# tomershay100/mp3-steganography-lib

Measured on AMD Instinct MI355X. Metric: MP3 frames/sec (decode+re-encode) @44.1kHz stereo 128kbps, 1→8 GPU, higher is better.
Workload: dtype f64 (decode) / int32 (encode); 1 GPU; 10000-frame full decode->stego-embed->re-encode pipeline per MI355X (BASELINE configs[2]); MP3 main data + side info resident in HBM, MP3 frames out; the message cursor chain is decided and the serial chains of the rate loop are checked on the device inside every step; frames_per_gpu=10000, channels=2, message_bits=536, chain_verdict_units_to_redo=0, message_variant_entries=1874, parallelism=frames sharded over 1 GPU(s), no collective

## Files before the change

include/mp3s.h:

```cpp
#ifndef MP3S_H
#define MP3S_H
#include <stddef.h>
#include <stdint.h>

#ifdef __cplusplus
extern "C" {
#endif

#define MP3S_OK 0
#define MP3S_E_NO_DEVICE (-1)
#define MP3S_E_HIP (-2)
#define MP3S_E_ARG (-3)
#define MP3S_E_MALFORMED (-4)
#define MP3S_E_UNSUPPORTED (-5)
#define MP3S_E_STEP_RANGE (-6)
#define MP3S_E_NOMEM (-7)
#define MP3S_E_EXIT (-8)
#define MP3S_E_BUSY (-9)
#define MP3S_E_TABLES (-10)

#define MP3S_PCM_I16 0
#define MP3S_PCM_F32 1
#define MP3S_PCM_F64 2

// ... 95 lines not shown
int mp3s_debug_walk_rate(const uint8_t *file, size_t len, double seconds, double *frames_per_s, int64_t *frames_per_pass);

int mp3s_dev_alloc(mp3s_ctx *ctx, size_t bytes, void **dptr);
int mp3s_dev_free(mp3s_ctx *ctx, void *dptr);
int mp3s_dev_upload(mp3s_ctx *ctx, void *dptr, const void *host, size_t bytes);
int mp3s_dev_download(mp3s_ctx *ctx, void *host, const void *dptr, size_t bytes);
int mp3s_dev_memset(mp3s_ctx *ctx, void *dptr, int value, size_t bytes);
int mp3s_dev_copy(mp3s_ctx *ctx, void *d_dst, const void *d_src, size_t bytes);
int mp3s_timer_start(mp3s_ctx *ctx);
int mp3s_timer_stop(mp3s_ctx *ctx, float *ms);
int mp3s_synth_mode(mp3s_ctx *ctx, double eps_scale, int64_t *exact_samples);
int mp3s_bench_copy(mp3s_ctx *ctx, size_t bytes, int iters, double *gb_per_s);
#define MP3S_N_KERNELS 9
#define MP3S_N_KERNELS_MIN 8
int mp3s_profile_enable(mp3s_ctx *ctx, int on);
int mp3s_profile_select(mp3s_ctx *ctx, unsigned mask);
int mp3s_profile_collect(mp3s_ctx *ctx, double *total_ms, int64_t *launches, int n);

int mp3s_decode_transform_dev(mp3s_ctx *ctx, const int16_t *d_is, const mp3s_granule_si *d_si,
                              const mp3s_frame_hdr *d_hdr, int n_frames, int nch, int n_halo, int out_format,
                              void *d_pcm);
int mp3s_decode_transform(mp3s_ctx *ctx, const int16_t *is, const mp3s_granule_si *si, const mp3s_frame_hdr *hdr,
                          int n_frames, int nch, int n_halo, int out_format, void *pcm);

int mp3s_encode_transform_dev(mp3s_ctx *ctx, const int16_t *d_pcm, const mp3s_frame_hdr *d_hdr, int n_frames,
                              int32_t *d_mdct);
int mp3s_encode_transform(mp3s_ctx *ctx, const int16_t *pcm, const mp3s_frame_hdr *hdr, int n_frames,
                          int32_t *mdct);

int mp3s_rate_loop_dev(mp3s_ctx *ctx, const int32_t *d_mdct, const mp3s_rate_frame *d_frames, int n_frames,
                       const uint8_t *d_hide_bits, int n_hide, const int32_t *d_cursor_in, const int32_t *d_state_in,
                       const int32_t *d_unit_list, int n_list, int16_t *d_ix, mp3s_gr_out *d_out, int32_t *d_en);

typedef struct {
    int32_t first_frame, n_frames;
    int32_t hide_base;
    int32_t hide_begin;
    int32_t hide_end;
    int32_t reserved;
    int32_t chain_in[4][4];
} mp3s_chain_seg;
typedef struct {
    int64_t cursor;
    int32_t chain[4][4];
    int32_t carry_used;
    int32_t reserved;
} mp3s_chain_seg_out;
int mp3s_chain_resolve_dev(mp3s_ctx *ctx, mp3s_gr_out *d_gr, const mp3s_rate_frame *d_frames, int n_frames,
                           const mp3s_chain_seg *d_segs, int n_segs, const int32_t *d_cursor_in, const int32_t *d_state_in,
                           int32_t *d_verdict, mp3s_chain_seg_out *d_seg_out);

int mp3s_chain_redo_dev(mp3s_ctx *ctx, const int32_t *d_mdct, const mp3s_rate_frame *d_frames, int n_frames,
                        const uint8_t *d_hide_bits, int n_hide, int32_t *d_cursor, const mp3s_chain_seg *d_segs, int n_segs,
                        int16_t *d_ix, mp3s_gr_out *d_gr, int32_t *d_en, int32_t *d_verdict, mp3s_chain_seg_out *d_seg_out);

#define MP3S_SELECT_VARIANTS 10
#define MP3S_SELECT_TAIL_FIRST(bits_left, reach) ((bits_left) < 2 ? 0 : (((bits_left) - 2) / 3 < (reach) ? ((bits_left) - 2) / 3 : (reach)))
#define MP3S_SELECT_ENTRIES(bits_left, reach) (8 * (reach) + 2 * ((reach) - MP3S_SELECT_TAIL_FIRST(bits_left, reach)))
#define MP3S_SELECT_MAX_REACH (1 << 18)
#define MP3S_NO_CURSOR 0x3fffffff
typedef struct {
    int32_t first_entry;
    int32_t reach;
} mp3s_select_span;
void mp3s_select_patterns(uint8_t out[32]);
int mp3s_select_plan(const mp3s_chain_seg *segs, int n_segs, mp3s_select_span *spans, int32_t *ent_unit, int32_t *ent_cursor, int cap);
// ... 298 lines not shown
```

mp3-steganography-lib_amd/csrc/k_chain.hpp:

```cpp
#pragma once

namespace mp3s {

constexpr int CH_THREADS = 256;

struct ChainEl { int reset, tables, last[4]; };

__device__ __forceinline__ ChainEl chain_identity() { return ChainEl{0, 0, {-1, -1, -1, -1}}; }
__device__ __forceinline__ ChainEl chain_combine(const ChainEl &l, const ChainEl &r)
{
    if (r.reset) return r;
    ChainEl o;
    o.reset = l.reset;
    o.tables = l.tables + r.tables;
#pragma unroll
    for (int k = 0; k < 4; k++) o.last[k] = r.last[k] >= 0 ? r.last[k] : l.last[k];
    return o;
}
__device__ __forceinline__ ChainEl chain_shfl_up(const ChainEl &x, int d)
{
    ChainEl o;
    o.reset = __shfl_up(x.reset, d, 64);
    o.tables = __shfl_up(x.tables, d, 64);
#pragma unroll
    for (int k = 0; k < 4; k++) o.last[k] = __shfl_up(x.last[k], d, 64);
    return o;
}

__device__ __forceinline__ ChainEl chain_block_scan(ChainEl x, ChainEl (&wave_tot)[CH_THREADS / 64], ChainEl *total)
{
    const int lane = threadIdx.x & 63, wave = threadIdx.x >> 6;
#pragma unroll
    for (int d = 1; d < 64; d <<= 1) {
        const ChainEl o = chain_shfl_up(x, d);
        if (lane >= d) x = chain_combine(o, x);
    }
    __syncthreads();
    if (lane == 63) wave_tot[wave] = x;
    __syncthreads();
    ChainEl pre = chain_identity();
#pragma unroll
    for (int w = 0; w < CH_THREADS / 64; w++) {
        if (w < wave) pre = chain_combine(pre, wave_tot[w]);
    }
    x = chain_combine(pre, x);
    if (total) {
        ChainEl t = wave_tot[0];
#pragma unroll
        for (int w = 1; w < CH_THREADS / 64; w++) t = chain_combine(t, wave_tot[w]);
        *total = t;
    }
    return x;
}

__device__ __forceinline__ ChainEl chain_element(const mp3s_gr_out *__restrict__ gr, const mp3s_rate_frame *__restrict__ rf,
                                                 const mp3s_chain_seg *__restrict__ segs, int f, int n_frames)
{
    ChainEl e = chain_identity();
    if (f >= n_frames) return e;
    e.reset = segs[rf[f].stream].first_frame == f ? 1 : 0;
#pragma unroll
    for (int k = 0; k < 4; k++) {
        const mp3s_gr_out &g = gr[(long)f * 4 + k];
        if (g.flags & MP3S_RF_ACTIVE) { e.tables += g.n_tables; e.last[k] = f * 4 + k; }
    }
    return e;
}

__global__ __launch_bounds__(CH_THREADS) void k_chain_sum(const mp3s_gr_out *__restrict__ gr, const mp3s_rate_frame *__restrict__ rf,
                                                          const mp3s_chain_seg *__restrict__ segs, int n_frames,
                                                          ChainEl *__restrict__ agg, int32_t *__restrict__ verdict,
                                                          mp3s_chain_seg_out *__restrict__ seg_out, int32_t *__restrict__ redo,
                                                          const int32_t *__restrict__ only_after)
{
    __shared__ ChainEl wave_tot[CH_THREADS / 64];
    if (only_after && only_after[0] == 0) {
        if (redo && blockIdx.x == 0 && threadIdx.x == 0) redo[0] = 0;
        return;
    }
    const int f = blockIdx.x * CH_THREADS + threadIdx.x;
    if (f == 0) { verdict[0] = 0; verdict[1] = 0; }
    if (redo) {
        if (f == 0) redo[0] = 0;
        if (f == 0 && !only_after) redo[REDO_WORDS] = 0;
    }
    if (f < n_frames && segs[rf[f].stream].first_frame == f) seg_out[rf[f].stream].carry_used = 0;
    ChainEl total;
    chain_block_scan(chain_element(gr, rf, segs, f, n_frames), wave_tot, &total);
    if (threadIdx.x == 0) agg[blockIdx.x] = total;
}

__global__ __launch_bounds__(CH_THREADS) void k_chain_apply(mp3s_gr_out *__restrict__ gr, const mp3s_rate_frame *__restrict__ rf,
                                                            const mp3s_chain_seg *__restrict__ segs, int n_frames,
                                                            const ChainEl *__restrict__ agg, int32_t *__restrict__ cursor_in,
                                                            const int32_t *__restrict__ state_in, int32_t *__restrict__ verdict,
                                                            mp3s_chain_seg_out *__restrict__ seg_out, int32_t *__restrict__ redo_list,
                                                            const int32_t *__restrict__ only_after)
{
    if (only_after && only_after[0] == 0) return;
    __shared__ ChainEl wave_tot[CH_THREADS / 64];
    const int f = blockIdx.x * CH_THREADS + threadIdx.x;
    ChainEl before = chain_identity();
    for (int c0 = 0; c0 < (int)blockIdx.x; c0 += CH_THREADS) {
        const int j = c0 + (int)threadIdx.x;
        ChainEl total;
        chain_block_scan(j < (int)blockIdx.x ? agg[j] : chain_identity(), wave_tot, &total);
        before = chain_combine(before, total);
    }
    const ChainEl own_el = chain_element(gr, rf, segs, f, n_frames);
    const ChainEl incl = chain_block_scan(own_el, wave_tot, nullptr);
    ChainEl excl = chain_shfl_up(incl, 1);
    if ((threadIdx.x & 63) == 0) {
        excl = chain_identity();
        for (int w = 0; w < (int)(threadIdx.x >> 6); w++) excl = chain_combine(excl, wave_tot[w]);
    }
    excl = chain_combine(before, excl);
    int redo_here = 0, err_here = 0;
    if (f < n_frames) {
        const int s = rf[f].stream;
        const mp3s_chain_seg sg = segs[s];
        const bool first = sg.first_frame == f;
        if (first) excl = chain_identity();
        long cur = (long)sg.hide_begin + excl.tables;
        const long end = sg.hide_end;
        const bool hiding = sg.hide_end > sg.hide_base;
        int carry_used = first && cur < end ? 1 : 0;
#pragma unroll
        for (int k = 0; k < 4; k++) {
            const long u = (long)f * 4 + k;
            mp3s_gr_out &g = gr[u];
            int32_t ch[4];
            const bool own = excl.last[k] >= 0;
            if (own) {
                const mp3s_gr_out &p = gr[excl.last[k]];
                ch[0] = p.address[0]; ch[1] = p.address[1]; ch[2] = p.address[2]; ch[3] = p.quantizer_step;
            } else {
#pragma unroll
                for (int j = 0; j < 4; j++) ch[j] = sg.chain_in[k][j];
            }
            const int flags = g.flags;
            const bool active = flags & MP3S_RF_ACTIVE;
            if (!own && (!active || (flags & MP3S_RF_USED_ADDR_IN))) carry_used = 1;
            bool redo = false;
            if (hiding && active) {
                const long used = cursor_in[u];
                if (used != cur && (used < cur ? used : cur) < end) redo = true;
            }
            if (flags & MP3S_RF_USED_ADDR_IN) {
                const int32_t given = state_in ? state_in[u * 4] | (state_in[u * 4 + 1] << 10) | (state_in[u * 4 + 2] << 20) : g.reserved0;
                if (given != (ch[0] | (ch[1] << 10) | (ch[2] << 20))) redo = true;
            }
            redo_here += redo ? 1 : 0;
            if (redo && redo_list) {
                const int at = atomicAdd(&redo_list[0], 1);
                if (at < REDO_CAP) {
                    const int32_t c = (int32_t)(cur < (long)MP3S_NO_CURSOR ? cur : (long)MP3S_NO_CURSOR);
                    redo_list[REDO_HEAD + at] = (int32_t)u;
                    g.flags = flags | MP3S_RF_LISTED;
                    redo_list[REDO_HEAD + REDO_CAP + at] = hiding ? c : (cursor_in ? cursor_in[u] : 0);
                    if (hiding) cursor_in[u] = c;
#pragma unroll
                    for (int j = 0; j < 4; j++) redo_list[REDO_HEAD + 2 * REDO_CAP + 4 * at + j] = ch[j];
                }
            } else if (flags & MP3S_RF_LISTED) {
                g.flags = flags & ~MP3S_RF_LISTED;
            }
            if (flags & MP3S_RF_STEP_RANGE) err_here = 1;
            if (active) cur += g.n_tables;
            else {
                g.address[0] = ch[0]; g.address[1] = ch[1]; g.address[2] = ch[2];
                g.quantizer_step = ch[3];
            }
        }
        if (carry_used) atomicOr(&seg_out[s].carry_used, 1);
        if (f == sg.first_frame + sg.n_frames - 1) {
            seg_out[s].cursor = cur;
#pragma unroll
            for (int k = 0; k < 4; k++) {
                const mp3s_gr_out &g = gr[(long)f * 4 + k];
                seg_out[s].chain[k][0] = g.address[0]; seg_out[s].chain[k][1] = g.address[1];
                seg_out[s].chain[k][2] = g.address[2]; seg_out[s].chain[k][3] = g.quantizer_step;
            }
        }
    }
    const int n_redo = (int)wave_add_u32((uint32_t)redo_here);
    const bool any_err = __ballot(err_here != 0) != 0;
    if ((threadIdx.x & 63) == 0) {
        if (n_redo) atomicAdd(&verdict[0], n_redo);
        if (any_err) atomicOr(&verdict[1], 1);
    }
}

constexpr int SEL_THREADS = 1024, SEL_WAVES = SEL_THREADS / 64, SEL_D = 128;
constexpr int SEL_ROUND = SEL_THREADS;
constexpr int SEL_SAFE = 32;
constexpr int SEL_NONE = MP3S_SELECT_VARIANTS;

__host__ __device__ inline size_t select_lds_bytes(int reach)
{
    const int rs = reach < SEL_ROUND ? reach : SEL_ROUND;
    return (size_t)rs * (SEL_NONE + 1) + (size_t)(3 * rs + SEL_D + 8) + (size_t)rs + SEL_WAVES * SEL_D + 64;
}

__global__ __launch_bounds__(SEL_THREADS) void k_chain_select(const mp3s_chain_seg *__restrict__ segs, const mp3s_select_span *__restrict__ spans,
                                                              int max_reach, const uint8_t *__restrict__ hide,
                                                              const uint8_t *__restrict__ tabv, const mp3s_gr_out *__restrict__ out,
                                                              int32_t *__restrict__ cursor, int2 *__restrict__ pairs)
{
    extern __shared__ uint8_t sel_lds[];
    __shared__ int overflow, d_next, d_try, sat_round;
    const int s = blockIdx.x;
    const mp3s_select_span sp = spans[s];
    const int R = sp.reach;
    const int tid = threadIdx.x, lane = tid & 63, wave = __builtin_amdgcn_readfirstlane(tid >> 6);
    int2 *my_pairs = pairs + (long)s * max_reach;
    if (R <= 0) {
        for (int j = tid; j < max_reach; j += SEL_THREADS) my_pairs[j] = make_int2(-1, 0);
        return;
    }
    const mp3s_chain_seg sg = segs[s];
    const long c0 = sg.hide_begin, end = sg.hide_end;
    const long u0 = (long)sg.first_frame * 4;
    const int RS = min(R, SEL_ROUND);
    const long left = end - c0;
    const int tail = (int)MP3S_SELECT_TAIL_FIRST(left, (long)R), R2 = R - tail;
    const long row8 = (long)sp.first_entry + 8L * R - tail;
    uint8_t *tabs = sel_lds;
    uint8_t *code = tabs + (size_t)RS * (SEL_NONE + 1);
    uint8_t *delta = code + 3 * RS + SEL_D + 8;
    uint8_t *tot = delta + RS;
    if (tid == 0) { overflow = 0; d_next = 0; }
    int size = SEL_ROUND;
    for (int J = 0; J < R;) {
        __syncthreads();
        if (tid == 0) sat_round = 0;
        const int Rs = min(size, R - J);
        const int d0 = d_next;
        const long rel0 = 3L * J - d0 - (SEL_D - 1);
        if (c0 + rel0 >= end) {
            for (int jj = tid; jj < Rs; jj += SEL_THREADS) my_pairs[J + jj] = make_int2(-1, 0);
// ... 38 lines not shown
                d = step(jj, d);
            }
            if (sat && lane == 0) sat_round = 1;
            if (wave == SEL_WAVES - 1 && lane == 0) d_try = d0 + d;
        }
        __syncthreads();
        if (sat_round) {
            if (size > SEL_SAFE) { size = SEL_SAFE; continue; }
            if (tid == 0) overflow = 1;
        }
        for (int jj = tid; jj < Rs; jj += SEL_THREADS) {
            const int p = 3 * jj + (SEL_D - 1) - (int)delta[jj];
            const int v = code[p];
            const int j = J + jj;
            if (v >= 8 && v != SEL_NONE && j < tail) overflow = 1;
            my_pairs[j] = v == SEL_NONE ? make_int2(-1, 0)
                                        : make_int2(v < 8 ? sp.first_entry + v * R + j : (int)(row8 + (long)(v - 8) * R2 + j), (int)(rel0 + p));
        }
        if (tid == 0) d_next = d_try;
        J += Rs;
        if (size == SEL_SAFE && J % SEL_ROUND == 0) size = SEL_ROUND;
    }
    __syncthreads();
    const bool bad = overflow != 0;
    for (int j = tid; j < max_reach; j += SEL_THREADS) {
        int src = -1;
        if (j < R && !bad) {
            const int2 pr = my_pairs[j];
            src = pr.x;
            if (src >= 0) cursor[u0 + j] = (int32_t)(c0 + pr.y);
        }
        my_pairs[j] = make_int2(src, (int)(u0 + j));
    }
}

}
```

mp3-steganography-lib_amd/csrc/k_rate.hpp:

```cpp
#pragma once
#ifndef MP3S_RL_STATS
#define MP3S_RL_STATS 0
#endif
#ifndef MP3S_RL_OCC
#define MP3S_RL_OCC 6
#endif
#if MP3S_RL_STATS
__device__ unsigned long long g_rl_stats[128];
extern "C" __attribute__((visibility("default"))) int mp3s_debug_rl_stats(unsigned long long *out, int clear)
{
    (void)hipDeviceSynchronize();
    int rc = (int)hipMemcpyFromSymbol(out, HIP_SYMBOL(g_rl_stats), sizeof(unsigned long long) * 128);
    if (clear) { unsigned long long z[128] = {}; rc |= (int)hipMemcpyToSymbol(HIP_SYMBOL(g_rl_stats), z, sizeof z); }
    return rc;
}
#define RL_STAT(i, v) do { if ((threadIdx.x & 63) == 0) atomicAdd(&g_rl_stats[(i)], (unsigned long long)(v)); } while (0)
#define RL_CLK() __builtin_readcyclecounter()
#else
#define RL_STAT(i, v) do { } while (0)
#endif

namespace mp3s {

#define RL_DPP(v, ctrl, rm) ((uint32_t)__builtin_amdgcn_update_dpp(0, (int)(v), ctrl, rm, 0xf, false))
// ... 610 lines not shown
        if (!CHAIN) break;
        ch_state[0] = __builtin_amdgcn_readfirstlane(st.a1); ch_state[1] = __builtin_amdgcn_readfirstlane(st.a2);
        ch_state[2] = __builtin_amdgcn_readfirstlane(st.a3); ch_state[3] = __builtin_amdgcn_readfirstlane(qstep);
        bool go = false;
        int un = u;
        for (;;) {
            un += 4;
            if (++steps >= REDO_CHAIN_MAX || un >= n_units || frames[un >> 2].stream != fr.stream) break;
            const int f2 = __builtin_amdgcn_readfirstlane(__hip_atomic_load(&out[un - out_base].flags, __ATOMIC_RELAXED, __HIP_MEMORY_SCOPE_AGENT));
            if (f2 & MP3S_RF_LISTED) break;
            if (!(f2 & MP3S_RF_ACTIVE)) continue;
            const int given = __builtin_amdgcn_readfirstlane(__hip_atomic_load(&out[un - out_base].reserved0, __ATOMIC_RELAXED, __HIP_MEMORY_SCOPE_AGENT));
            go = (f2 & MP3S_RF_USED_ADDR_IN) && given != (ch_state[0] | (ch_state[1] << 10) | (ch_state[2] << 20));
            break;
        }
        if (!go) break;
        u = un; chained = true;
        ch_cursor = (n_hide_all > 0 && cursor_all) ? cursor_all[u] : 0;
    }
    }
    } while (CHAIN && (li0 += (int)gridDim.x * RL_WAVES) < n_total);
}

__global__ __launch_bounds__(RL_WAVES * 64, MP3S_RL_OCC) void k_rate_loop(
    const int32_t *__restrict__ mdct, const mp3s_rate_frame *__restrict__ frames, int n_units,
    const uint8_t *__restrict__ hide, int n_hide, const int32_t *__restrict__ cursor_in,
    const int32_t *__restrict__ state_in, const int32_t *__restrict__ unit_list, int n_list,
    int16_t *__restrict__ ix_out, mp3s_gr_out *__restrict__ out, int32_t *__restrict__ en_out, int out_base, int compact,
    RateVariants var)
{
    rate_units(mdct, frames, n_units, hide, n_hide, cursor_in, state_in, unit_list, n_list, ix_out, out, en_out, out_base, compact, var);
}

__global__ __launch_bounds__(RL_WAVES * 64, 4) void k_rate_redo(
    const int32_t *__restrict__ mdct, const mp3s_rate_frame *__restrict__ frames, int n_units,
    const uint8_t *__restrict__ hide, int n_hide, const int32_t *__restrict__ redo, int16_t *__restrict__ ix_out,
    mp3s_gr_out *__restrict__ out, int32_t *__restrict__ en_out, const int32_t *__restrict__ cursor_all)
{
    const int32_t *unit_list = redo + REDO_HEAD;
    const int n_list = min(__builtin_amdgcn_readfirstlane(__hip_atomic_load(&redo[0], __ATOMIC_RELAXED, __HIP_MEMORY_SCOPE_AGENT)), REDO_CAP);
    if ((int)blockIdx.x * RL_WAVES >= n_list) return;
    const RateVariants none = {nullptr, nullptr, 0, nullptr, nullptr, nullptr, nullptr};
    rate_units<true>(mdct, frames, n_units, hide, n_hide, unit_list + REDO_CAP, unit_list + 2 * REDO_CAP, unit_list, n_list, ix_out, out, en_out,
                  0, 3, none, cursor_all);
}

__global__ __launch_bounds__(256) void k_gather_tables(const mp3s_gr_out *__restrict__ outv, int n, uint8_t *__restrict__ tables)
{
    const int i = blockIdx.x * 256 + threadIdx.x;
    if (i < n) tables[i] = (uint8_t)outv[i].n_tables;
}

__global__ __launch_bounds__(256) void k_scatter_entries(const int2 *__restrict__ pairs, int n_pairs, const int16_t *__restrict__ ixv,
                                                         const int32_t *__restrict__ env, const mp3s_gr_out *__restrict__ outv,
                                                         int16_t *__restrict__ ix, int32_t *__restrict__ en, mp3s_gr_out *__restrict__ out)
{
    const int wave = __builtin_amdgcn_readfirstlane(threadIdx.x >> 6), lane = threadIdx.x & 63;
    const int j = blockIdx.x * 4 + wave;
    if (j >= n_pairs) return;
    const int2 pr = pairs[j];
    if (pr.x < 0) return;
    const long src = pr.x, dst = pr.y;
    const uint32_t *a = reinterpret_cast<const uint32_t *>(ixv + src * 576);
    uint32_t *b = reinterpret_cast<uint32_t *>(ix + dst * 576);
    for (int i = lane; i < 288; i += 64) b[i] = a[i];
    if (lane < 22) en[dst * 22 + lane] = env[src * 22 + lane];
    static_assert(sizeof(mp3s_gr_out) % 4 == 0, "GrInfo is copied by words");
    if (lane < (int)(sizeof(mp3s_gr_out) / 4))
        reinterpret_cast<uint32_t *>(out + dst)[lane] = reinterpret_cast<const uint32_t *>(outv + src)[lane];
}

}
```

mp3-steganography-lib_amd/csrc/mp3s_device.hip:

```cpp
#include <hip/hip_runtime.h>
#include <hip/hip_ext.h>
#include <atomic>
#include <stdint.h>
#include <stdlib.h>

#include "../../include/mp3s.h"
#include "mp3s_device.h"
#include "mp3s_host.h"
#include "mp3s_tables.h"

namespace mp3s {
__constant__ DevTables c_tab;
}

#include "k_sync.hpp"
#include "k_decode.hpp"
#include "k_decode_stream.hpp"
#include "k_encode.hpp"
#include "k_rate.hpp"
#include "k_huffman.hpp"
#include "k_parse.hpp"
#include "k_reveal.hpp"
#include "k_capacity.hpp"
#include "k_pack.hpp"
// ... 164 lines not shown
    hipLaunchKernelGGL(k_enc_analysis, dim3((unsigned)((waves + 3) / 4)), dim3(256), 0, stream, d_pcm, d_hdr, n_frames, SB,
                       Ts);
    if (prof) prof->end(stream, pp);
    pp = prof ? prof->begin(stream, K_ENC_MDCT) : -1;
    hipLaunchKernelGGL(k_enc_mdct, dim3((n_frames + 3) / 4), dim3(256), 0, stream, (const int32_t *)SB, Ts, d_hdr, n_frames,
                       d_mdct);
    if (prof) prof->end(stream, pp);
    return (int)hipGetLastError();
}

int launch_rate(hipStream_t stream, const int32_t *d_mdct, const mp3s_rate_frame *d_frames, int n_frames,
                const uint8_t *d_hide, int n_hide, const int32_t *d_cursor, const int32_t *d_state,
                const int32_t *d_list, int n_list, int16_t *d_ix, mp3s_gr_out *d_out, int32_t *d_en, Profiler *prof, int out_base, int compact,
                const RateVariantArgs *variants, hipEvent_t done)
{
    const int n_units = n_frames * 4;
    if (compact && !d_list) return (int)hipErrorInvalidValue;
    const int n = d_list ? n_list : n_units;
    RateVariants var = {nullptr, nullptr, 0, nullptr, nullptr, nullptr, nullptr};
    if (variants && variants->n > 0) var = RateVariants{variants->d_unit, variants->d_cursor, variants->n, variants->d_ix, variants->d_out, variants->d_en, variants->d_tables};
    if (n + var.n <= 0) return done ? (int)hipEventRecord(done, stream) : 0;
    hipEvent_t t_start = nullptr, t_stop = nullptr;
    const bool timed = prof && prof->attach(K_RATE_LOOP, &t_start, &t_stop);
    if (timed || done)
        hipExtLaunchKernelGGL(k_rate_loop, dim3((n + var.n + RL_WAVES - 1) / RL_WAVES), dim3(RL_WAVES * 64), 0, stream, timed ? t_start : nullptr, timed ? t_stop : done, 0,
                              d_mdct, d_frames, n_units, d_hide, n_hide, d_cursor, d_state, d_list, n, d_ix, d_out, d_en, out_base, compact, var);
    else
        hipLaunchKernelGGL(k_rate_loop, dim3((n + var.n + RL_WAVES - 1) / RL_WAVES), dim3(RL_WAVES * 64), 0, stream, d_mdct, d_frames,
                           n_units, d_hide, n_hide, d_cursor, d_state, d_list, n, d_ix, d_out, d_en, out_base, compact, var);
    if (timed && done && hipEventRecord(done, stream) != hipSuccess) return (int)hipErrorUnknown;
    return (int)hipGetLastError();
}

static size_t chain_scan_bytes(int n_frames) { return ((size_t)((n_frames + CH_THREADS - 1) / CH_THREADS) * sizeof(ChainEl) + 31) & ~(size_t)15; }
constexpr int kRedoRounds = 1;
size_t chain_agg_bytes(int n_frames) { return chain_scan_bytes(n_frames) + (size_t)2 * REDO_WORDS * 4; }

int launch_chain(hipStream_t stream, mp3s_gr_out *d_gr, const mp3s_rate_frame *d_frames, int n_frames, const mp3s_chain_seg *d_segs,
                 const int32_t *d_cursor, const int32_t *d_state, void *d_agg, int32_t *d_verdict, mp3s_chain_seg_out *d_seg_out,
                 Profiler *prof, const ChainRedoArgs *redo)
{
    if (n_frames <= 0) return 0;
    const int blocks = (n_frames + CH_THREADS - 1) / CH_THREADS;
    int32_t *d_redo = redo ? (int32_t *)((uint8_t *)d_agg + chain_scan_bytes(n_frames)) : nullptr;
    int32_t *cursor = const_cast<int32_t *>(d_cursor);
    const int pp = prof ? prof->begin(stream, K_CHAIN) : -1;
    hipLaunchKernelGGL(k_chain_sum, dim3(blocks), dim3(CH_THREADS), 0, stream, (const mp3s_gr_out *)d_gr, d_frames, d_segs, n_frames,
                       (ChainEl *)d_agg, d_verdict, d_seg_out, d_redo, (const int32_t *)nullptr);
    hipLaunchKernelGGL(k_chain_apply, dim3(blocks), dim3(CH_THREADS), 0, stream, d_gr, d_frames, d_segs, n_frames,
                       (const ChainEl *)d_agg, cursor, d_state, d_verdict, d_seg_out, d_redo, (const int32_t *)nullptr);
    if (redo) {
        int32_t *lists[2] = {d_redo, d_redo + REDO_WORDS};
        for (int round = 0; round < kRedoRounds; round++) {
            const int32_t *cur = lists[round & 1];
            int32_t *nxt = round + 1 < kRedoRounds ? lists[(round + 1) & 1] : nullptr;
            hipLaunchKernelGGL(k_rate_redo, dim3(REDO_GROUPS), dim3(RL_WAVES * 64), 0, stream, redo->d_mdct, d_frames, n_frames * 4,
                               redo->d_hide, redo->n_hide, cur, redo->d_ix, d_gr, redo->d_en, (const int32_t *)d_cursor);
            hipLaunchKernelGGL(k_chain_sum, dim3(blocks), dim3(CH_THREADS), 0, stream, (const mp3s_gr_out *)d_gr, d_frames, d_segs, n_frames,
                               (ChainEl *)d_agg, d_verdict, d_seg_out, nxt, cur);
            hipLaunchKernelGGL(k_chain_apply, dim3(blocks), dim3(CH_THREADS), 0, stream, d_gr, d_frames, d_segs, n_frames,
                               (const ChainEl *)d_agg, cursor, d_state, d_verdict, d_seg_out, nxt, cur);
        }
    }
    if (prof) prof->end(stream, pp);
    return (int)hipGetLastError();
}

int launch_select(hipStream_t stream, const mp3s_chain_seg *d_segs, const mp3s_select_span *d_spans, int n_segs, int max_reach,
                  const uint8_t *d_hide, const RateVariantArgs &v, int16_t *d_ix, int32_t *d_en, mp3s_gr_out *d_out, int32_t *d_cursor,
                  void *d_pairs, Profiler *prof)
{
    if (n_segs <= 0 || max_reach <= 0 || v.n <= 0) return 0;
    if (max_reach > MP3S_SELECT_MAX_REACH || (int64_t)n_segs * max_reach > 0x3fffffff) return (int)hipErrorInvalidValue;
    const int pp = prof ? prof->begin(stream, K_CHAIN) : -1;
    hipLaunchKernelGGL(k_chain_select, dim3(n_segs), dim3(SEL_THREADS), select_lds_bytes(max_reach), stream, d_segs, d_spans, max_reach,
                       d_hide, (const uint8_t *)v.d_tables, (const mp3s_gr_out *)d_out, d_cursor, (int2 *)d_pairs);
    const int n_pairs = n_segs * max_reach;
    hipLaunchKernelGGL(k_scatter_entries, dim3((n_pairs + 3) / 4), dim3(256), 0, stream, (const int2 *)d_pairs, n_pairs,
                       (const int16_t *)v.d_ix, (const int32_t *)v.d_en, (const mp3s_gr_out *)v.d_out, d_ix, d_en, d_out);
    if (prof) prof->end(stream, pp);
    return (int)hipGetLastError();
}

int launch_gather_tables(hipStream_t stream, const mp3s_gr_out *d_outv, int n, uint8_t *d_tables)
{
    if (n <= 0) return 0;
    hipLaunchKernelGGL(k_gather_tables, dim3((n + 255) / 256), dim3(256), 0, stream, d_outv, n, d_tables);
    return (int)hipGetLastError();
}

int launch_scatter(hipStream_t stream, const int32_t *d_pairs, int n_pairs, const int16_t *d_ixv, const int32_t *d_env,
                   const mp3s_gr_out *d_outv, int16_t *d_ix, int32_t *d_en, mp3s_gr_out *d_out)
{
    if (n_pairs <= 0) return 0;
    hipLaunchKernelGGL(k_scatter_entries, dim3((n_pairs + 3) / 4), dim3(256), 0, stream, (const int2 *)d_pairs, n_pairs, d_ixv, d_env,
                       d_outv, d_ix, d_en, d_out);
    return (int)hipGetLastError();
}

int launch_huffman(hipStream_t stream, const uint8_t *d_blob, const mp3s_frame_side *d_side, int n_frames, int nch, int max_bits,
                   int16_t *d_is, mp3s_granule_si *d_si, int32_t *d_status, int32_t *d_sync, Profiler *prof, bool per_frame, int lanes_opt)
{
    const long units = (long)n_frames * 4;
    const int W = huf_words_for(max_bits);
    int dev = 0;
    (void)hipGetDevice(&dev);
    const int dslot = dev >= 0 && dev < 64 ? dev : 0;
    static std::atomic<int> lds_of_device[64];
    int lds_max = lds_of_device[dslot].load(std::memory_order_relaxed);
    if (lds_max == 0) {
        if (hipDeviceGetAttribute(&lds_max, hipDeviceAttributeMaxSharedMemoryPerBlock, dev) != hipSuccess || lds_max < 64 * 1024) lds_max = 64 * 1024;
        lds_of_device[dslot].store(lds_max, std::memory_order_relaxed);
// ... 169 lines not shown
```

Before: 19.58 million frames/s.

## Fuse chain scan into single-pass decoupled look-back kernel and fold redo check

Replaces the two-kernel chain prefix scan (per-block sum, then apply) with one kernel that uses decoupled look-back over generation-tagged slots. The last-arriving block reduces per-block records into the verdict. The redo rate pass now ends with a last-block arrival and a serial chain check inside the same kernel instead of re-launching the sum and apply kernels. The select step can also copy entries itself, skipping the scatter kernel when reach is small. This cuts kernel launches and global round trips per step, at the cost of spin-polling, atomics, a fallback path for incomplete look-back, and more complex memory-ordering correctness.

```diff
diff --git a/include/mp3s.h b/include/mp3s.h
--- a/include/mp3s.h
+++ b/include/mp3s.h
@@ -151,6 +151,7 @@
                        const uint8_t *d_hide_bits, int n_hide, const int32_t *d_cursor_in, const int32_t *d_state_in,
                        const int32_t *d_unit_list, int n_list, int16_t *d_ix, mp3s_gr_out *d_out, int32_t *d_en);
 
+#define MP3S_CHAIN_INCOMPLETE 0x40000000
 typedef struct {
     int32_t first_frame, n_frames;
     int32_t hide_base;
diff --git a/mp3-steganography-lib_amd/csrc/k_chain.hpp b/mp3-steganography-lib_amd/csrc/k_chain.hpp
--- a/mp3-steganography-lib_amd/csrc/k_chain.hpp
+++ b/mp3-steganography-lib_amd/csrc/k_chain.hpp
@@ -1,22 +1,10 @@
 #pragma once
+#include "k_chain_scan.hpp"
 
 namespace mp3s {
 
 constexpr int CH_THREADS = 256;
 
-struct ChainEl { int reset, tables, last[4]; };
-
-__device__ __forceinline__ ChainEl chain_identity() { return ChainEl{0, 0, {-1, -1, -1, -1}}; }
-__device__ __forceinline__ ChainEl chain_combine(const ChainEl &l, const ChainEl &r)
-{
-    if (r.reset) return r;
-    ChainEl o;
-    o.reset = l.reset;
-    o.tables = l.tables + r.tables;
-#pragma unroll
-    for (int k = 0; k < 4; k++) o.last[k] = r.last[k] >= 0 ? r.last[k] : l.last[k];
-    return o;
-}
 __device__ __forceinline__ ChainEl chain_shfl_up(const ChainEl &x, int d)
 {
     ChainEl o;
@@ -26,6 +14,15 @@
     for (int k = 0; k < 4; k++) o.last[k] = __shfl_up(x.last[k], d, 64);
     return o;
 }
+__device__ __forceinline__ ChainEl chain_shfl_down(const ChainEl &x, int d)
+{
+    ChainEl o;
+    o.reset = __shfl_down(x.reset, d, 64);
+    o.tables = __shfl_down(x.tables, d, 64);
+#pragma unroll
+    for (int k = 0; k < 4; k++) o.last[k] = __shfl_down(x.last[k], d, 64);
+    return o;
+}
 
 __device__ __forceinline__ ChainEl chain_block_scan(ChainEl x, ChainEl (&wave_tot)[CH_THREADS / 64], ChainEl *total)
 {
@@ -67,58 +64,126 @@
     return e;
 }
 
-__global__ __launch_bounds__(CH_THREADS) void k_chain_sum(const mp3s_gr_out *__restrict__ gr, const mp3s_rate_frame *__restrict__ rf,
-                                                          const mp3s_chain_seg *__restrict__ segs, int n_frames,
-                                                          ChainEl *__restrict__ agg, int32_t *__restrict__ verdict,
-                                                          mp3s_chain_seg_out *__restrict__ seg_out, int32_t *__restrict__ redo,
-                                                          const int32_t *__restrict__ only_after)
-{
-    __shared__ ChainEl wave_tot[CH_THREADS / 64];
-    if (only_after && only_after[0] == 0) {
-        if (redo && blockIdx.x == 0 && threadIdx.x == 0) redo[0] = 0;
-        return;
-    }
-    const int f = blockIdx.x * CH_THREADS + threadIdx.x;
-    if (f == 0) { verdict[0] = 0; verdict[1] = 0; }
-    if (redo) {
-        if (f == 0) redo[0] = 0;
-        if (f == 0 && !only_after) redo[REDO_WORDS] = 0;
-    }
-    if (f < n_frames && segs[rf[f].stream].first_frame == f) seg_out[rf[f].stream].carry_used = 0;
-    ChainEl total;
-    chain_block_scan(chain_element(gr, rf, segs, f, n_frames), wave_tot, &total);
-    if (threadIdx.x == 0) agg[blockIdx.x] = total;
-}
-
-__global__ __launch_bounds__(CH_THREADS) void k_chain_apply(mp3s_gr_out *__restrict__ gr, const mp3s_rate_frame *__restrict__ rf,
-                                                            const mp3s_chain_seg *__restrict__ segs, int n_frames,
-                                                            const ChainEl *__restrict__ agg, int32_t *__restrict__ cursor_in,
-                                                            const int32_t *__restrict__ state_in, int32_t *__restrict__ verdict,
-                                                            mp3s_chain_seg_out *__restrict__ seg_out, int32_t *__restrict__ redo_list,
-                                                            const int32_t *__restrict__ only_after)
-{
-    if (only_after && only_after[0] == 0) return;
-    __shared__ ChainEl wave_tot[CH_THREADS / 64];
-    const int f = blockIdx.x * CH_THREADS + threadIdx.x;
-    ChainEl before = chain_identity();
-    for (int c0 = 0; c0 < (int)blockIdx.x; c0 += CH_THREADS) {
-        const int j = c0 + (int)threadIdx.x;
-        ChainEl total;
-        chain_block_scan(j < (int)blockIdx.x ? agg[j] : chain_identity(), wave_tot, &total);
-        before = chain_combine(before, total);
-    }
-    const ChainEl own_el = chain_element(gr, rf, segs, f, n_frames);
-    const ChainEl incl = chain_block_scan(own_el, wave_tot, nullptr);
+__device__ __forceinline__ unsigned tagged_add(unsigned long long *w, unsigned gen, unsigned add)
+{
+    unsigned long long old = __hip_atomic_load(w, __ATOMIC_RELAXED, __HIP_MEMORY_SCOPE_AGENT);
+    for (;;) {
+        const unsigned cnt = (unsigned)(old >> 32) == gen ? (unsigned)old : 0u;
+        const unsigned long long seen = atomicCAS(w, old, ((unsigned long long)gen << 32) | (cnt + add));
+        if (seen == old) return cnt;
+        old = seen;
+    }
+}
+__device__ __forceinline__ unsigned tagged_count(const unsigned long long *w, unsigned gen)
+{
+    const unsigned long long v = __hip_atomic_load(w, __ATOMIC_RELAXED, __HIP_MEMORY_SCOPE_AGENT);
+    return (unsigned)(v >> 32) == gen ? (unsigned)v : 0u;
+}
+
+__device__ __forceinline__ bool chain_arrive(unsigned long long *w, unsigned gen, unsigned n_groups, int *flag )
+{
+    asm volatile("s_waitcnt vmcnt(0)" ::: "memory");
+    __syncthreads();
+    if (threadIdx.x == 0) {
+        __builtin_amdgcn_fence(__ATOMIC_RELEASE, "agent");
+        asm volatile("s_waitcnt vmcnt(0)" ::: "memory");
+        const bool last = tagged_add(w, gen, 1u) + 1u == n_groups;
+        if (last) {
+            __builtin_amdgcn_fence(__ATOMIC_ACQUIRE, "agent");
+            asm volatile("s_waitcnt vmcnt(0)" ::: "memory");
+        }
+        *flag = last ? 1 : 0;
+    }
+    __syncthreads();
+    return *flag != 0;
+}
+
+struct ChainRecord { int32_t redo, bits, seg_in, reserved; };
+constexpr int CHR_STEP_RANGE = 1, CHR_INCOMPLETE = 2, CHR_CARRY_IN = 4;
+constexpr size_t CH_HEAD_BYTES = 128;
+__host__ __device__ inline size_t chain_slots_bytes(int blocks) { return (size_t)blocks * CH_SLOT_WORDS * 8; }
+__host__ __device__ inline size_t chain_scan_bytes_for(int blocks) { return CH_HEAD_BYTES + chain_slots_bytes(blocks) + (size_t)blocks * sizeof(ChainRecord); }
+
+struct ChainDevWindow {
+    const unsigned long long *slots;
+    unsigned gen;
+    int lane;
+    ChainEl a, p;
+    bool va, vp, vg;
+    __device__ __forceinline__ void read(int pos, int n)
+    {
+        va = vp = vg = false;
+        a = chain_identity(); p = chain_identity();
+        if (lane < n) {
+            const unsigned long long *q = slots + (long)(pos - lane) * CH_SLOT_WORDS;
+            unsigned long long ga[CH_FIELDS], gp[CH_FIELDS];
+#pragma unroll
+            for (int k = 0; k < CH_FIELDS; k++) {
+                ga[k] = __hip_atomic_load(q + CH_SLOT_AGG + k, __ATOMIC_RELAXED, __HIP_MEMORY_SCOPE_AGENT);
+                gp[k] = __hip_atomic_load(q + CH_SLOT_PREFIX + k, __ATOMIC_RELAXED, __HIP_MEMORY_SCOPE_AGENT);
+            }
+            vg = chain_granule_is(__hip_atomic_load(q + CH_SLOT_GIVEN_UP, __ATOMIC_RELAXED, __HIP_MEMORY_SCOPE_AGENT), gen);
+            va = vp = true;
+#pragma unroll
+            for (int k = 0; k < CH_FIELDS; k++) {
+                va = va && chain_granule_is(ga[k], gen);
+                vp = vp && chain_granule_is(gp[k], gen);
+                chain_set_field(a, k, (int32_t)(uint32_t)ga[k]);
+                chain_set_field(p, k, (int32_t)(uint32_t)gp[k]);
+            }
+        }
+    }
+    __device__ __forceinline__ uint64_t prefix_mask() const { return __ballot(vp); }
+    __device__ __forceinline__ uint64_t aggregate_mask() const { return __ballot(va); }
+    __device__ __forceinline__ uint64_t given_up_mask() const { return __ballot(vg); }
+    __device__ __forceinline__ ChainEl fold(int n_agg, bool prefix) const
+    {
+        ChainEl x = lane < n_agg ? a : (prefix && lane == n_agg ? p : chain_identity());
+#pragma unroll
+        for (int d = 1; d < 64; d <<= 1) {
+            const ChainEl o = chain_shfl_down(x, d);
+            if (lane + d < 64) x = chain_combine(o, x);
+        }
+        ChainEl r;
+        r.reset = __shfl(x.reset, 0, 64);
+        r.tables = __shfl(x.tables, 0, 64);
+#pragma unroll
+        for (int k = 0; k < 4; k++) r.last[k] = __shfl(x.last[k], 0, 64);
+        return r;
+    }
+    __device__ __forceinline__ void pause() const { __builtin_amdgcn_s_sleep(8); }
+};
+
+__device__ __forceinline__ void chain_publish(unsigned long long *words, const ChainEl &e, unsigned gen, int lane)
+{
+    if (lane < CH_FIELDS) __hip_atomic_store(words + lane, chain_granule(gen, chain_field(e, lane)), __ATOMIC_RELAXED, __HIP_MEMORY_SCOPE_AGENT);
+}
+
+struct ChainTally { int redo, err, carry_in, seg_in; };
+template <bool SERIAL>
+__device__ __forceinline__ ChainTally chain_apply(mp3s_gr_out *__restrict__ gr, const mp3s_rate_frame *__restrict__ rf,
+                                                  const mp3s_chain_seg *__restrict__ segs, int n_frames, int f, int chunk_first,
+                                                  const ChainEl &before, const ChainEl &incl, const ChainEl (&wave_tot)[CH_THREADS / 64],
+                                                  int32_t *__restrict__ cursor_in, const int32_t *__restrict__ state_in,
+                                                  mp3s_chain_seg_out *__restrict__ seg_out, int32_t *__restrict__ redo_list, unsigned gen)
+{
+    ChainTally t = {0, 0, 0, 0};
     ChainEl excl = chain_shfl_up(incl, 1);
     if ((threadIdx.x & 63) == 0) {
         excl = chain_identity();
         for (int w = 0; w < (int)(threadIdx.x >> 6); w++) excl = chain_combine(excl, wave_tot[w]);
     }
     excl = chain_combine(before, excl);
-    int redo_here = 0, err_here = 0;
+    int s = 0;
+    mp3s_chain_seg sg = {};
     if (f < n_frames) {
-        const int s = rf[f].stream;
-        const mp3s_chain_seg sg = segs[s];
+        s = rf[f].stream;
+        sg = segs[s];
+        if (sg.first_frame == f) atomicExch(&seg_out[s].carry_used, 0);
+    }
+    asm volatile("s_waitcnt vmcnt(0)" ::: "memory");
+    __syncthreads();
+    if (f < n_frames) {
         const bool first = sg.first_frame == f;
         if (first) excl = chain_identity();
         long cur = (long)sg.hide_begin + excl.tables;
@@ -138,7 +203,8 @@
 #pragma unroll
                 for (int j = 0; j < 4; j++) ch[j] = sg.chain_in[k][j];
             }
-            const int flags = g.flags;
+            const int flags_was = g.flags;
+            int flags = flags_was & ~MP3S_RF_LISTED;
             const bool active = flags & MP3S_RF_ACTIVE;
             if (!own && (!active || (flags & MP3S_RF_USED_ADDR_IN))) carry_used = 1;
             bool redo = false;
@@ -150,29 +216,31 @@
                 const int32_t given = state_in ? state_in[u * 4] | (state_in[u * 4 + 1] << 10) | (state_in[u * 4 + 2] << 20) : g.reserved0;
                 if (given != (ch[0] | (ch[1] << 10) | (ch[2] << 20))) redo = true;
             }
-            redo_here += redo ? 1 : 0;
+            t.redo += redo ? 1 : 0;
             if (redo && redo_list) {
-                const int at = atomicAdd(&redo_list[0], 1);
+                const int at = (int)tagged_add(reinterpret_cast<unsigned long long *>(redo_list), gen, 1u);
                 if (at < REDO_CAP) {
                     const int32_t c = (int32_t)(cur < (long)MP3S_NO_CURSOR ? cur : (long)MP3S_NO_CURSOR);
                     redo_list[REDO_HEAD + at] = (int32_t)u;
-                    g.flags = flags | MP3S_RF_LISTED;
+                    flags |= MP3S_RF_LISTED;
                     redo_list[REDO_HEAD + REDO_CAP + at] = hiding ? c : (cursor_in ? cursor_in[u] : 0);
                     if (hiding) cursor_in[u] = c;
 #pragma unroll
                     for (int j = 0; j < 4; j++) redo_list[REDO_HEAD + 2 * REDO_CAP + 4 * at + j] = ch[j];
                 }
-            } else if (flags & MP3S_RF_LISTED) {
-                g.flags = flags & ~MP3S_RF_LISTED;
-            }
-            if (flags & MP3S_RF_STEP_RANGE) err_here = 1;
+            }
+            if (flags != flags_was) g.flags = flags;
+            if (flags & MP3S_RF_STEP_RANGE) t.err = 1;
             if (active) cur += g.n_tables;
             else {
                 g.address[0] = ch[0]; g.address[1] = ch[1]; g.address[2] = ch[2];
                 g.quantizer_step = ch[3];
             }
         }
-        if (carry_used) atomicOr(&seg_out[s].carry_used, 1);
+        if (carry_used) {
+            if (SERIAL || sg.first_frame >= chunk_first) atomicOr(&seg_out[s].carry_used, 1);
+            else { t.carry_in = 1; t.seg_in = s; }
+        }
         if (f == sg.first_frame + sg.n_frames - 1) {
             seg_out[s].cursor = cur;
 #pragma unroll
@@ -183,12 +251,111 @@
             }
         }
     }
-    const int n_redo = (int)wave_add_u32((uint32_t)redo_here);
-    const bool any_err = __ballot(err_here != 0) != 0;
+    return t;
+}
+
+__device__ __forceinline__ void chain_tally_add(const ChainTally &t, int *sums)
+{
+    const int n_redo = (int)wave_add_u32((uint32_t)t.redo);
+    const bool any_err = __ballot(t.err != 0) != 0;
+    const uint64_t in = __ballot(t.carry_in != 0);
     if ((threadIdx.x & 63) == 0) {
-        if (n_redo) atomicAdd(&verdict[0], n_redo);
-        if (any_err) atomicOr(&verdict[1], 1);
-    }
+        if (n_redo) atomicAdd(&sums[0], n_redo);
+        if (any_err) atomicOr(&sums[1], CHR_STEP_RANGE);
+    }
+    if (in && (int)(threadIdx.x & 63) == __ffsll((long long)in) - 1) { atomicOr(&sums[1], CHR_CARRY_IN); sums[2] = t.seg_in; }
+}
+
+__global__ __launch_bounds__(CH_THREADS) void k_chain_check(mp3s_gr_out *__restrict__ gr, const mp3s_rate_frame *__restrict__ rf,
+                                                            const mp3s_chain_seg *__restrict__ segs, int n_frames,
+                                                            unsigned long long *__restrict__ scratch, unsigned gen, int poll_budget,
+                                                            int32_t *__restrict__ cursor_in, const int32_t *__restrict__ state_in,
+                                                            int32_t *__restrict__ verdict, mp3s_chain_seg_out *__restrict__ seg_out,
+                                                            int32_t *__restrict__ redo_list)
+{
+    __shared__ ChainEl wave_tot[CH_THREADS / 64];
+    __shared__ ChainEl before_s;
+    __shared__ int look_s, last_s, sums[3];
+    const int b = blockIdx.x, blocks = gridDim.x, lane = threadIdx.x & 63, wave = threadIdx.x >> 6;
+    const int f = b * CH_THREADS + (int)threadIdx.x;
+    unsigned long long *slots = scratch + CH_HEAD_BYTES / 8, *mine = slots + (long)b * CH_SLOT_WORDS;
+    ChainRecord *records = reinterpret_cast<ChainRecord *>(slots + (long)blocks * CH_SLOT_WORDS);
+    if (threadIdx.x == 0) { sums[0] = 0; sums[1] = 0; sums[2] = 0; }
+    ChainEl total;
+    const ChainEl incl = chain_block_scan(chain_element(gr, rf, segs, f, n_frames), wave_tot, &total);
+    if (wave == 0) {
+        const bool early = b == 0 || total.reset != 0;
+        chain_publish(mine + (early ? CH_SLOT_PREFIX : CH_SLOT_AGG), total, gen, lane);
+        ChainEl before = chain_identity();
+        int look = CHAIN_LOOK_OK;
+        if (b > 0) {
+            ChainDevWindow win = {slots, gen, lane, chain_identity(), chain_identity(), false, false, false};
+            look = chain_look_back(win, b, poll_budget, &before);
+            if (look == CHAIN_LOOK_OK) {
+                if (!early) chain_publish(mine + CH_SLOT_PREFIX, chain_combine(before, total), gen, lane);
+            } else if (!early && lane == 0)
+                __hip_atomic_store(mine + CH_SLOT_GIVEN_UP, chain_granule(gen, 1), __ATOMIC_RELAXED, __HIP_MEMORY_SCOPE_AGENT);
+        }
+        if (lane == 0) { before_s = before; look_s = look; }
+    }
+    __syncthreads();
+    const bool complete = look_s == CHAIN_LOOK_OK;
+    if (complete) {
+        const ChainEl before = before_s;
+        const ChainTally t = chain_apply<false>(gr, rf, segs, n_frames, f, b * CH_THREADS, before, incl, wave_tot, cursor_in, state_in, seg_out, redo_list, gen);
+        chain_tally_add(t, sums);
+    }
+    __syncthreads();
+    if (threadIdx.x == 0) records[b] = ChainRecord{sums[0], sums[1] | (complete ? 0 : CHR_INCOMPLETE), sums[2], 0};
+    if (!chain_arrive(scratch, gen, (unsigned)blocks, &last_s)) return;
+    if (threadIdx.x == 0) { sums[0] = 0; sums[1] = 0; }
+    __syncthreads();
+    int redo = 0, bits = 0;
+    for (int j = threadIdx.x; j < blocks; j += CH_THREADS) {
+        const ChainRecord r = records[j];
+        redo += r.redo;
+        bits |= r.bits;
+        if (r.bits & CHR_CARRY_IN) atomicOr(&seg_out[r.seg_in].carry_used, 1);
+    }
+    redo = (int)wave_add_u32((uint32_t)redo);
+    const bool err = __ballot((bits & CHR_STEP_RANGE) != 0) != 0, incomplete = __ballot((bits & CHR_INCOMPLETE) != 0) != 0;
+    if (lane == 0) {
+        if (redo) atomicAdd(&sums[0], redo);
+        if (err || incomplete) atomicOr(&sums[1], (err ? CHR_STEP_RANGE : 0) | (incomplete ? CHR_INCOMPLETE : 0));
+    }
+    __syncthreads();
+    if (threadIdx.x == 0) {
+        const bool inc = (sums[1] & CHR_INCOMPLETE) != 0;
+        verdict[0] = inc ? (sums[0] | MP3S_CHAIN_INCOMPLETE) : sums[0];
+        verdict[1] = (sums[1] & CHR_STEP_RANGE) ? 1 : 0;
+        if (inc && redo_list) *reinterpret_cast<unsigned long long *>(redo_list) = 0ull;
+    }
+}
+
+__device__ __noinline__ void chain_check_serial(mp3s_gr_out *__restrict__ gr, const mp3s_rate_frame *__restrict__ rf,
+                                                const mp3s_chain_seg *__restrict__ segs, int n_frames, int32_t *__restrict__ cursor_in,
+                                                int32_t *__restrict__ verdict, mp3s_chain_seg_out *__restrict__ seg_out)
+{
+    __shared__ ChainEl wave_tot[CH_THREADS / 64];
+    __shared__ int sums[3];
+    if (threadIdx.x == 0) { sums[0] = 0; sums[1] = 0; sums[2] = 0; }
+    ChainEl before = chain_identity();
+    ChainTally all = {0, 0, 0, 0};
+    for (int c0 = 0; c0 < n_frames; c0 += CH_THREADS) {
+        const int f = c0 + (int)threadIdx.x;
+        ChainEl total;
+        const ChainEl incl = chain_block_scan(chain_element(gr, rf, segs, f, n_frames), wave_tot, &total);
+        const ChainTally t = chain_apply<true>(gr, rf, segs, n_frames, f, c0, before, incl, wave_tot, cursor_in, nullptr, seg_out, nullptr, 0u);
+        all.redo += t.redo;
+        all.err |= t.err;
+        before = chain_combine(before, total);
+        asm volatile("s_waitcnt vmcnt(0)" ::: "memory");
+        __syncthreads();
+    }
+    __syncthreads();
+    chain_tally_add(all, sums);
+    __syncthreads();
+    if (threadIdx.x == 0) { verdict[0] = sums[0]; verdict[1] = (sums[1] & CHR_STEP_RANGE) ? 1 : 0; }
 }
 
 constexpr int SEL_THREADS = 1024, SEL_WAVES = SEL_THREADS / 64, SEL_D = 128;
@@ -202,10 +369,12 @@
     return (size_t)rs * (SEL_NONE + 1) + (size_t)(3 * rs + SEL_D + 8) + (size_t)rs + SEL_WAVES * SEL_D + 64;
 }
 
+constexpr int SEL_COPY_MAX = 1024;
+struct SelectCopy { const int16_t *ixv; const int32_t *env; const mp3s_gr_out *outv; int16_t *ix; int32_t *en; int own_copy; };
 __global__ __launch_bounds__(SEL_THREADS) void k_chain_select(const mp3s_chain_seg *__restrict__ segs, const mp3s_select_span *__restrict__ spans,
                                                               int max_reach, const uint8_t *__restrict__ hide,
-                                                              const uint8_t *__restrict__ tabv, const mp3s_gr_out *__restrict__ out,
-                                                              int32_t *__restrict__ cursor, int2 *__restrict__ pairs)
+                                                              const uint8_t *__restrict__ tabv, mp3s_gr_out *out,
+                                                              int32_t *__restrict__ cursor, int2 *pairs, SelectCopy cp)
 {
     extern __shared__ uint8_t sel_lds[];
     __shared__ int overflow, d_next, d_try, sat_round;
@@ -310,6 +479,20 @@
         }
         my_pairs[j] = make_int2(src, (int)(u0 + j));
     }
-}
-
-}
+    if (!cp.own_copy) return;
+    asm volatile("s_waitcnt vmcnt(0)" ::: "memory");
+    __syncthreads();
+    for (int j = wave; j < R; j += SEL_WAVES) {
+        const int2 pr = my_pairs[j];
+        if (pr.x < 0) continue;
+        const long src = pr.x, dst = pr.y;
+        const uint32_t *a = reinterpret_cast<const uint32_t *>(cp.ixv + src * 576);
+        uint32_t *b = reinterpret_cast<uint32_t *>(cp.ix + dst * 576);
+        for (int i = lane; i < 288; i += 64) b[i] = a[i];
+        if (lane < 22) cp.en[dst * 22 + lane] = cp.env[src * 22 + lane];
+        if (lane < (int)(sizeof(mp3s_gr_out) / 4))
+            reinterpret_cast<uint32_t *>(out + dst)[lane] = reinterpret_cast<const uint32_t *>(cp.outv + src)[lane];
+    }
+}
+
+}
diff --git a/mp3-steganography-lib_amd/csrc/k_chain_scan.hpp b/mp3-steganography-lib_amd/csrc/k_chain_scan.hpp
--- /dev/null
+++ b/mp3-steganography-lib_amd/csrc/k_chain_scan.hpp
@@ -0,0 +1,74 @@
+#pragma once
+#include <stdint.h>
+
+#if defined(__HIPCC__)
+#define CHAIN_HD __host__ __device__ __forceinline__
+#else
+#define CHAIN_HD inline
+#endif
+
+namespace mp3s {
+
+struct ChainEl { int reset, tables, last[4]; };
+
+CHAIN_HD ChainEl chain_identity() { return ChainEl{0, 0, {-1, -1, -1, -1}}; }
+CHAIN_HD ChainEl chain_combine(const ChainEl &l, const ChainEl &r)
+{
+    if (r.reset) return r;
+    ChainEl o;
+    o.reset = l.reset;
+    o.tables = l.tables + r.tables;
+    for (int k = 0; k < 4; k++) o.last[k] = r.last[k] >= 0 ? r.last[k] : l.last[k];
+    return o;
+}
+CHAIN_HD int chain_field(const ChainEl &e, int k)
+{
+    return k == 0 ? e.reset : k == 1 ? e.tables : k == 2 ? e.last[0] : k == 3 ? e.last[1] : k == 4 ? e.last[2] : e.last[3];
+}
+CHAIN_HD void chain_set_field(ChainEl &e, int k, int v)
+{
+    if (k == 0) e.reset = v;
+    else if (k == 1) e.tables = v;
+    else if (k == 2) e.last[0] = v;
+    else if (k == 3) e.last[1] = v;
+    else if (k == 4) e.last[2] = v;
+    else e.last[3] = v;
+}
+
+constexpr int CH_SLOT_WORDS = 16, CH_SLOT_AGG = 0, CH_SLOT_GIVEN_UP = 6, CH_SLOT_PREFIX = 8, CH_FIELDS = 6;
+constexpr int CH_WINDOW = 64;
+constexpr int CH_POLL_BUDGET = 4096;
+constexpr int CHAIN_LOOK_OK = 0, CHAIN_LOOK_INCOMPLETE = 1;
+
+CHAIN_HD uint64_t chain_granule(uint32_t tag, int32_t v) { return ((uint64_t)tag << 32) | (uint32_t)v; }
+CHAIN_HD bool chain_granule_is(uint64_t g, uint32_t tag) { return (uint32_t)(g >> 32) == tag; }
+
+template <class Win>
+CHAIN_HD int chain_look_back(Win &win, int b, int budget, ChainEl *excl)
+{
+    ChainEl acc = chain_identity();
+    int pos = b - 1, polls = 0;
+    while (pos >= 0) {
+        const int n = pos + 1 < CH_WINDOW ? pos + 1 : CH_WINDOW;
+        win.read(pos, n);
+        const uint64_t in_win = n >= 64 ? ~(uint64_t)0 : (((uint64_t)1 << n) - 1);
+        const uint64_t mp = win.prefix_mask() & in_win, ma = win.aggregate_mask() & in_win, mg = win.given_up_mask() & in_win;
+        const uint64_t stop_mask = (mp | mg | ~ma) & in_win;
+        int stop = n;
+        if (stop_mask) { stop = 0; while (!((stop_mask >> stop) & 1)) stop++; }
+        const bool prefix = stop < n && ((mp >> stop) & 1);
+        if (stop < n && !prefix && ((mg >> stop) & 1)) return CHAIN_LOOK_INCOMPLETE;
+        if (stop > 0 || prefix) acc = chain_combine(win.fold(stop, prefix), acc);
+        if (prefix) break;
+        pos -= stop;
+        if (stop == n) continue;
+        if (stop == 0) {
+            if (polls++ >= budget) return CHAIN_LOOK_INCOMPLETE;
+            win.pause();
+        }
+    }
+    *excl = acc;
+    return CHAIN_LOOK_OK;
+}
+
+}
diff --git a/mp3-steganography-lib_amd/csrc/k_rate.hpp b/mp3-steganography-lib_amd/csrc/k_rate.hpp
--- a/mp3-steganography-lib_amd/csrc/k_rate.hpp
+++ b/mp3-steganography-lib_amd/csrc/k_rate.hpp
@@ -666,17 +666,28 @@
     rate_units(mdct, frames, n_units, hide, n_hide, cursor_in, state_in, unit_list, n_list, ix_out, out, en_out, out_base, compact, var);
 }
 
+__device__ __forceinline__ unsigned tagged_count(const unsigned long long *w, unsigned gen);
+__device__ __forceinline__ bool chain_arrive(unsigned long long *w, unsigned gen, unsigned n_groups, int *flag);
+__device__ void chain_check_serial(mp3s_gr_out *__restrict__ gr, const mp3s_rate_frame *__restrict__ rf, const mp3s_chain_seg *__restrict__ segs,
+                                   int n_frames, int32_t *__restrict__ cursor_in, int32_t *__restrict__ verdict,
+                                   mp3s_chain_seg_out *__restrict__ seg_out);
+struct RedoCheckArgs { unsigned gen; unsigned long long *arrive; const mp3s_chain_seg *segs; int32_t *verdict; mp3s_chain_seg_out *seg_out; };
+
 __global__ __launch_bounds__(RL_WAVES * 64, 4) void k_rate_redo(
     const int32_t *__restrict__ mdct, const mp3s_rate_frame *__restrict__ frames, int n_units,
     const uint8_t *__restrict__ hide, int n_hide, const int32_t *__restrict__ redo, int16_t *__restrict__ ix_out,
-    mp3s_gr_out *__restrict__ out, int32_t *__restrict__ en_out, const int32_t *__restrict__ cursor_all)
-{
+    mp3s_gr_out *__restrict__ out, int32_t *__restrict__ en_out, int32_t *__restrict__ cursor_all, RedoCheckArgs chk)
+{
+    __shared__ int last_s;
     const int32_t *unit_list = redo + REDO_HEAD;
-    const int n_list = min(__builtin_amdgcn_readfirstlane(__hip_atomic_load(&redo[0], __ATOMIC_RELAXED, __HIP_MEMORY_SCOPE_AGENT)), REDO_CAP);
+    const int n_list = min((int)__builtin_amdgcn_readfirstlane(tagged_count(reinterpret_cast<const unsigned long long *>(redo), chk.gen)), REDO_CAP);
     if ((int)blockIdx.x * RL_WAVES >= n_list) return;
     const RateVariants none = {nullptr, nullptr, 0, nullptr, nullptr, nullptr, nullptr};
     rate_units<true>(mdct, frames, n_units, hide, n_hide, unit_list + REDO_CAP, unit_list + 2 * REDO_CAP, unit_list, n_list, ix_out, out, en_out,
                   0, 3, none, cursor_all);
+    const int working = min((int)gridDim.x, (n_list + RL_WAVES - 1) / RL_WAVES);
+    if (!chain_arrive(chk.arrive, chk.gen, (unsigned)working, &last_s)) return;
+    chain_check_serial(out, frames, chk.segs, n_units / 4, cursor_all, chk.verdict, chk.seg_out);
 }
 
 __global__ __launch_bounds__(256) void k_gather_tables(const mp3s_gr_out *__restrict__ outv, int n, uint8_t *__restrict__ tables)
diff --git a/mp3-steganography-lib_amd/csrc/mp3s_device.hip b/mp3-steganography-lib_amd/csrc/mp3s_device.hip
--- a/mp3-steganography-lib_amd/csrc/mp3s_device.hip
+++ b/mp3-steganography-lib_amd/csrc/mp3s_device.hip
@@ -220,9 +220,16 @@
     return (int)hipGetLastError();
 }
 
-static size_t chain_scan_bytes(int n_frames) { return ((size_t)((n_frames + CH_THREADS - 1) / CH_THREADS) * sizeof(ChainEl) + 31) & ~(size_t)15; }
-constexpr int kRedoRounds = 1;
-size_t chain_agg_bytes(int n_frames) { return chain_scan_bytes(n_frames) + (size_t)2 * REDO_WORDS * 4; }
+static size_t chain_scan_bytes(int n_frames) { return (chain_scan_bytes_for((n_frames + CH_THREADS - 1) / CH_THREADS) + 31) & ~(size_t)15; }
+size_t chain_agg_bytes(int n_frames) { return chain_scan_bytes(n_frames) + (size_t)REDO_WORDS * 4; }
+
+static unsigned next_chain_generation()
+{
+    static std::atomic<unsigned> gen{0};
+    unsigned g;
+    do g = gen.fetch_add(1u, std::memory_order_relaxed) + 1u; while (g == 0u);
+    return g;
+}
 
 int launch_chain(hipStream_t stream, mp3s_gr_out *d_gr, const mp3s_rate_frame *d_frames, int n_frames, const mp3s_chain_seg *d_segs,
                  const int32_t *d_cursor, const int32_t *d_state, void *d_agg, int32_t *d_verdict, mp3s_chain_seg_out *d_seg_out,
@@ -232,23 +239,15 @@
     const int blocks = (n_frames + CH_THREADS - 1) / CH_THREADS;
     int32_t *d_redo = redo ? (int32_t *)((uint8_t *)d_agg + chain_scan_bytes(n_frames)) : nullptr;
     int32_t *cursor = const_cast<int32_t *>(d_cursor);
+    unsigned long long *scratch = (unsigned long long *)d_agg;
+    const unsigned gen = next_chain_generation();
     const int pp = prof ? prof->begin(stream, K_CHAIN) : -1;
-    hipLaunchKernelGGL(k_chain_sum, dim3(blocks), dim3(CH_THREADS), 0, stream, (const mp3s_gr_out *)d_gr, d_frames, d_segs, n_frames,
-                       (ChainEl *)d_agg, d_verdict, d_seg_out, d_redo, (const int32_t *)nullptr);
-    hipLaunchKernelGGL(k_chain_apply, dim3(blocks), dim3(CH_THREADS), 0, stream, d_gr, d_frames, d_segs, n_frames,
-                       (const ChainEl *)d_agg, cursor, d_state, d_verdict, d_seg_out, d_redo, (const int32_t *)nullptr);
+    hipLaunchKernelGGL(k_chain_check, dim3(blocks), dim3(CH_THREADS), 0, stream, d_gr, d_frames, d_segs, n_frames, scratch, gen, CH_POLL_BUDGET,
+                       cursor, d_state, d_verdict, d_seg_out, d_redo);
     if (redo) {
-        int32_t *lists[2] = {d_redo, d_redo + REDO_WORDS};
-        for (int round = 0; round < kRedoRounds; round++) {
-            const int32_t *cur = lists[round & 1];
-            int32_t *nxt = round + 1 < kRedoRounds ? lists[(round + 1) & 1] : nullptr;
-            hipLaunchKernelGGL(k_rate_redo, dim3(REDO_GROUPS), dim3(RL_WAVES * 64), 0, stream, redo->d_mdct, d_frames, n_frames * 4,
-                               redo->d_hide, redo->n_hide, cur, redo->d_ix, d_gr, redo->d_en, (const int32_t *)d_cursor);
-            hipLaunchKernelGGL(k_chain_sum, dim3(blocks), dim3(CH_THREADS), 0, stream, (const mp3s_gr_out *)d_gr, d_frames, d_segs, n_frames,
-                               (ChainEl *)d_agg, d_verdict, d_seg_out, nxt, cur);
-            hipLaunchKernelGGL(k_chain_apply, dim3(blocks), dim3(CH_THREADS), 0, stream, d_gr, d_frames, d_segs, n_frames,
-                               (const ChainEl *)d_agg, cursor, d_state, d_verdict, d_seg_out, nxt, cur);
-        }
+        const RedoCheckArgs chk = {gen, scratch + 1, d_segs, d_verdict, d_seg_out};
+        hipLaunchKernelGGL(k_rate_redo, dim3(REDO_GROUPS), dim3(RL_WAVES * 64), 0, stream, redo->d_mdct, d_frames, n_frames * 4,
+                           redo->d_hide, redo->n_hide, (const int32_t *)d_redo, redo->d_ix, d_gr, redo->d_en, cursor, chk);
     }
     if (prof) prof->end(stream, pp);
     return (int)hipGetLastError();
@@ -261,11 +260,15 @@
     if (n_segs <= 0 || max_reach <= 0 || v.n <= 0) return 0;
     if (max_reach > MP3S_SELECT_MAX_REACH || (int64_t)n_segs * max_reach > 0x3fffffff) return (int)hipErrorInvalidValue;
     const int pp = prof ? prof->begin(stream, K_CHAIN) : -1;
+    const bool own_copy = max_reach <= SEL_COPY_MAX;
+    const SelectCopy cp = {(const int16_t *)v.d_ix, (const int32_t *)v.d_en, (const mp3s_gr_out *)v.d_out, d_ix, d_en, own_copy ? 1 : 0};
     hipLaunchKernelGGL(k_chain_select, dim3(n_segs), dim3(SEL_THREADS), select_lds_bytes(max_reach), stream, d_segs, d_spans, max_reach,
-                       d_hide, (const uint8_t *)v.d_tables, (const mp3s_gr_out *)d_out, d_cursor, (int2 *)d_pairs);
-    const int n_pairs = n_segs * max_reach;
-    hipLaunchKernelGGL(k_scatter_entries, dim3((n_pairs + 3) / 4), dim3(256), 0, stream, (const int2 *)d_pairs, n_pairs,
-                       (const int16_t *)v.d_ix, (const int32_t *)v.d_en, (const mp3s_gr_out *)v.d_out, d_ix, d_en, d_out);
+                       d_hide, (const uint8_t *)v.d_tables, d_out, d_cursor, (int2 *)d_pairs, cp);
+    if (!own_copy) {
+        const int n_pairs = n_segs * max_reach;
+        hipLaunchKernelGGL(k_scatter_entries, dim3((n_pairs + 3) / 4), dim3(256), 0, stream, (const int2 *)d_pairs, n_pairs,
+                           (const int16_t *)v.d_ix, (const int32_t *)v.d_en, (const mp3s_gr_out *)v.d_out, d_ix, d_en, d_out);
+    }
     if (prof) prof->end(stream, pp);
     return (int)hipGetLastError();
 }
```

Measured after the change: 19.77 million frames/s, median of 3. Within noise of the previous version (+1.0%).
